# Minys233/GCN-BMP

Hardware: AMD Instinct MI355X
Metric: drug-pairs/sec fwd+bwd, binary-DDI GGNN d=128 (higher is better)
Workload: dtype f32; 1 GPU; C2: full binary DDI set (544 drugs, 147696 pairs), GGNN 4-step d=128 tied + Nie co-attention (head 8, tanh) + MLP(32,16), fwd+bwd+Adam, 1024 pairs/GPU/step, every molecule instance encoded; the 144 batches of one epoch resident in HBM, cycled; layout=per-instance packed layout, whole 128-row tiles, pairs_per_gpu=1024, global_batch=1024, parallelism=dp1

## Files before the change

gcn-bmp_amd/bmp/_lib.py:

```python
from __future__ import annotations

import ctypes
import os
from ctypes import c_float, c_int, c_size_t, c_void_p

import torch

_HERE = os.path.dirname(os.path.abspath(__file__))
LIB_PATH = os.environ.get("BMP_LIB_PATH") or os.path.join(_HERE, "libbmp_hip.so")

_P, _I, _Z, _F = c_void_p, c_int, c_size_t, c_float

SIGNATURES = {
    "bmp_version": (_I, []),
    "bmp_tile_rows": (_I, []),
    "bmp_prof_start": (_I, [_I]),
    "bmp_prof_stop": (_I, [_P]),
    "bmp_prof_collect": (_I, [_P, _P, _P, _P, _P, _I]),
    "bmp_stream_create_low": (_I, [_P]),
    "bmp_stream_destroy": (_I, [_P]),
    "bmp_embed_fwd": (_I, [_P, _P, _I, _I, _I, _P, _P]),
    "bmp_embed_bwd_ws_floats": (_Z, [_I, _I, _I]),
    "bmp_embed_bwd": (_I, [_P, _P, _I, _I, _I, _P, _P, _Z, _P]),
    "bmp_msg_fwd": (_I, [_P, _I, _I, _I, _I, _P, _P, _P, _P, _P, _P, _P, _I, _P, _P, _P, _I, _P]),
    "bmp_msg_bwd_ws_floats": (_Z, [_I, _I, _I]),
    "bmp_msg_bwd": (_I, [_P, _I, _P, _I, _I, _P, _I, _I, _I, _I, _P, _P, _P, _P, _P, _P, _P, _P, _P, _P, _P, _P, _I, _P, _P, _P, _Z, _P, _P]),
    "bmp_gru_fwd": (_I, [_P, _P, _I, _I, _I, _P, _P, _P, _P, _P, _P, _P]),
    "bmp_gru_bwd_ws_floats": (_Z, [_I, _I]),
    "bmp_gru_bwd": (_I, [_P, _P, _P, _P, _P, _I, _I, _I, _P, _P, _P, _P, _P, _P, _P, _I, _P, _Z, _P, _P]),
    "bmp_gru_state_fwd": (_I, [_P, _P, _P, _I, _I] + [_P] * 8),
    "bmp_gru_state_bwd_ws_floats": (_Z, [_I, _I]),
    "bmp_gru_state_bwd": (_I, [_P, _P, _P, _P, _P, _P, _I, _I] + [_P] * 11 + [_Z, _P]),
    "bmp_ggnn_step_supported": (_I, [_I]),
    "bmp_ggnn_step_fwd": (_I, [_P, _I, _I, _I, _I] + [_P] * 14 + [_I, _I, _P]),
    "bmp_ggnn_step_bwd": (_I, [_P, _P, _P, _P, _I, _I, _I] + [_P] * 10 + [_I, _I, _I, _P]),
    "bmp_step_wgrad_lists_used": (_I, [_I, _I]),
    "bmp_ggnn_step_wgrad_ws_floats": (_Z, [_I, _I]),
    "bmp_ggnn_step_wgrad": (_I, [_P, _P, _P, _P, _I, _I, _I, _P, _P, _P, _P, _I, _P, _P, _P, _P, _P, _Z, _P]),
    "bmp_type_rows_ws_ints": (_Z, [_I]),
    "bmp_type_rows": (_I, [_P, _P, _I, _P, _P, _P, _P]),
    "bmp_type_rows_live": (_I, [_P, _P, _P, _I, _P, _P, _P, _P]),
    "bmp_readout_tile_supported": (_I, [_I, _I, _I]),
    "bmp_readout_tile_fwd": (_I, [_P, _P, _I, _I, _P, _P, _I, _P, _P, _P, _P, _P, _P]),
    "bmp_relgcn_layer_supported": (_I, [_I, _I]),
    "bmp_relgcn_layer_fwd": (_I, [_P, _I, _I, _I, _P, _P, _P, _P, _P, _P, _P, _I, _P, _P, _P, _P, _I, _P]),
    "bmp_relgcn_layer_bwd": (_I, [_P, _P, _I, _I, _I, _P, _P, _P, _P, _P, _P, _P, _P, _P, _I, _I, _P]),
    "bmp_relgcn_layer_wgrad_ws_floats": (_Z, [_I, _I]),
    "bmp_relgcn_layer_wgrad": (_I, [_P, _P, _P, _I, _I, _P, _P, _P, _I, _P, _P, _P, _Z, _P]),
    "bmp_readout_fwd": (_I, [_P, _P, _I, _I, _I, _I, _P, _P, _I, _P, _P, _P, _I, _P, _P, _P]),
    "bmp_readout_bwd_ws_floats": (_Z, [_I, _I, _I, _I]),
    "bmp_readout_bwd": (_I, [_P, _P, _P, _I, _I, _I, _I, _P, _P, _I, _P, _P, _P, _I, _P, _P, _P, _P, _I, _P, _Z, _P, _P]),
    "bmp_linear_fwd": (_I, [_P, _I, _I, _I, _I, _P, _I, _P, _I, _P, _I, _P]),
    "bmp_wgrad_ws_floats_c": (_Z, [_I, _I, _I]),
    "bmp_linear_wgrad": (_I, [_P, _I, _P, _I, _I, _I, _I, _P, _P, _P, _Z, _P]),
    "bmp_segpool_fwd": (_I, [_P, _I, _P, _I, _P, _P, _P, _I, _P, _P]),
    "bmp_segpool_bwd": (_I, [_P, _P, _I, _P, _I, _P, _P, _P, _I, _I, _P, _P, _P]),
    "bmp_segsoftmax_fwd": (_I, [_P, _P, _P, _P, _I, _I, _P, _P]),
    "bmp_segsoftmax_bwd": (_I, [_P, _P, _P, _P, _P, _I, _I, _P, _P]),
    "bmp_rowbcast_fwd": (_I, [_P, _I, _P, _I, _P, _P]),
    "bmp_rowbcast_bwd": (_I, [_P, _I, _P, _P, _I, _P, _P]),
    "bmp_rowdot_fwd": (_I, [_P, _I, _P, _P, _P, _I, _P, _P]),
    "bmp_rowdot_bwd": (_I, [_P, _P, _I, _P, _P, _P, _P, _I, _I, _P, _P, _P, _P]),
    "bmp_rowcorr_fwd": (_I, [_P, _I, _P, _P, _P, _I, _P, _P]),
    "bmp_rowcorr_bwd": (_I, [_P, _P, _I, _P, _P, _P, _I, _P, _P, _P]),
    "bmp_dense_count": (_I, [_P, _I, _I, _P, _P, _P]),
    "bmp_dense_to_csr": (_I, [_P, _I, _I, _P, _P, _I, _P, _P, _P]),
    "bmp_collate_plan": (_I, [_P, _P, _I, _P, _P, _I, _P, _I, _P, _P, _P]),
    "bmp_collate_pair_meta": (_I, [_P, _I, _I, _I, _I, _P, _P, _P]),
# ... 104 lines not shown
```

gcn-bmp_amd/bmp/functional.py:

```python
from __future__ import annotations

import os

import torch
from torch.autograd import Function

from . import _lib
from ._lib import check, ptr, stream, require_rows
from .packed import PackedMolBatch

ACT = {"identity": 0, None: 0, "sigmoid": 1, "tanh": 2, "relu": 3}


def _ws(nfloats: int, device) -> torch.Tensor:
    return torch.empty(max(int(nfloats), 4), dtype=torch.float32, device=device)


def _check_pb(pb: PackedMolBatch, x: torch.Tensor) -> None:
    L = _lib.lib()
    if pb.R != L.bmp_tile_rows():
        raise ValueError(f"packed batch tile size R={pb.R} != library tile rows {L.bmp_tile_rows()}")
    if x.shape[0] != pb.n_rows:
        raise ValueError(f"row tensor has {x.shape[0]} rows, packed batch has {pb.n_rows}")

# ... 169 lines not shown
    tr = pb.type_rows_T(forward=forward)
    return tr if tr is not None else (None, None)


def step_lists(pb, N: int, d: int):
    tri, trc = type_rows(pb)
    if tri is None or not _lib.lib().bmp_step_wgrad_lists_used(int(N), int(d)):
        return None, None, 0
    return tri, trc, 1


def _rel_mt(pb):
    return (None, None) if pb.tile_stride else (pb.mt_row0, pb.mt_nblk)


def step_supported(d: int) -> bool:
    return bool(_lib.lib().bmp_ggnn_step_supported(int(d)))


def pack_k4(W: torch.Tensor) -> torch.Tensor:
    K, N = W.shape
    return W.detach().reshape(K // 4, 4, N).permute(0, 2, 1).contiguous()


def _cached(cache, tag, src, make):
    if cache is None:
        return make()
    key = (tag, src.data_ptr())
    if key not in cache:
        cache[key] = (make(), src)
    return cache[key][0]


class GGNNStepFn(Function):

    @staticmethod
    def forward(ctx, h, WT, bE, AT, UcT, b, pb, first, cache=None):
        L = _lib.lib()
        require_rows(h, "step: h")
        _check_pb(pb, h)
        N, d = h.shape
        if tuple(WT.shape) != (4 * d, d) or tuple(bE.shape) != (4, d) or tuple(AT.shape) != (2 * d, 3 * d) \
                or tuple(UcT.shape) != (d, d) or tuple(b.shape) != (3 * d,):
            raise ValueError("step: weight shapes do not match h")
        bE, b = bE.contiguous(), b.contiguous()
        WTp = _cached(cache, "f", WT, lambda: pack_k4(WT))
        ATp = _cached(cache, "f", AT, lambda: pack_k4(AT))
        UcTp = _cached(cache, "f", UcT, lambda: pack_k4(UcT))
        f = lambda *s: torch.empty(*s, dtype=torch.float32, device=h.device)
        m, rz, c, hout = f(N, d), f(N, 2 * d), f(N, d), f(N, d)
        check(L.bmp_ggnn_step_fwd(ptr(h), 0, pb.n_mtiles, d, int(first), ptr(pb.csr_ptr), ptr(pb.csr_col), ptr(pb.csr_val),
                                  ptr(WTp), ptr(bE), ptr(ATp), ptr(UcTp), ptr(b), ptr(m), ptr(rz), ptr(c), ptr(hout),
                                  ptr(pb.mt_row0), ptr(pb.mt_nblk), pb.n_rows, pb.tile_stride, stream()), "bmp_ggnn_step_fwd")
        ctx.save_for_backward(h, WT, AT, UcT, m, rz, c)
        ctx.pb, ctx.first, ctx.cache = pb, int(first), cache
        if cache is not None:
            key = ("n", WT.data_ptr(), AT.data_ptr())
            cache[key] = cache.get(key, 0) + 1
        return hout

    @staticmethod
    def backward(ctx, dhout):
        L = _lib.lib()
        h, WT, AT, UcT, m, rz, c = ctx.saved_tensors
        pb, first, cache = ctx.pb, ctx.first, ctx.cache
        N, d = h.shape
        dev = h.device
        dhout = dhout.contiguous()
        Wnat = _cached(cache, "b", WT, lambda: pack_k4(WT.t()))
        A = _cached(cache, "b", AT, lambda: pack_k4(AT.t()))
        Uc = _cached(cache, "b", UcT, lambda: pack_k4(UcT.t()))
        f = lambda *s: torch.empty(*s, dtype=torch.float32, device=dev)
        dh, gda = f(N, d), f(N, 7 * d)
        tri, trc, skip = step_lists(pb, N, d)
        check(L.bmp_ggnn_step_bwd(ptr(dhout), ptr(h), ptr(rz), ptr(c), pb.n_mtiles, d, first, ptr(pb.csrT_ptr),
                                  ptr(pb.csrT_col), ptr(pb.csrT_val), ptr(Wnat), ptr(A), ptr(Uc), ptr(dh), ptr(gda),
                                  ptr(pb.mt_row0), ptr(pb.mt_nblk), pb.n_rows, pb.tile_stride, skip, stream()), "bmp_ggnn_step_bwd")
        grp = ("g", WT.data_ptr(), AT.data_ptr())
        st = None
        if cache is not None and cache.get(("n",) + grp[1:], 1) > 1:
            st = cache.setdefault(grp, dict(seen=0, buf=None))
        if st is None or st["buf"] is None:
            o1, o2, dUcT, cs = f(d, 7 * d), f(d, 3 * d), f(d, d), f(7 * d)
            if st is not None:
                st["buf"] = (o1, o2, dUcT, cs)
        else:
            o1, o2, dUcT, cs = st["buf"]
        acc = 1 if (st is not None and st["seen"] > 0) else 0
        nws = L.bmp_ggnn_step_wgrad_ws_floats(N, d)
        ws = _ws(nws, dev)
        check(L.bmp_ggnn_step_wgrad(ptr(h), ptr(m), ptr(rz), ptr(gda), N, d, first, ptr(o1), ptr(o2), ptr(dUcT), ptr(cs),
                                    acc, ptr(tri), ptr(trc), None, None, ptr(ws), nws, stream()), "bmp_ggnn_step_wgrad")
        if st is not None:
            st["seen"] += 1
            if st["seen"] < cache[("n",) + grp[1:]]:
                return dh, None, None, None, None, None, None, None, None
            st["seen"], st["buf"] = 0, None
        dWT = o1[:, :4 * d].reshape(d, 4, d).permute(1, 0, 2).reshape(4 * d, d)
        dbE = cs[:4 * d].reshape(4, d)
        dAT = torch.cat((o1[:, 4 * d:], o2), dim=0)
        return dh, dWT, dbE, dAT, dUcT, cs[4 * d:], None, None, None


def flush_deferred_bwd(state) -> None:
    if state is not None and state.get("deferred_bwd"):
        fns = state["deferred_bwd"]
        state["deferred_bwd"] = []
        for fn in fns:
            fn()


def flush_deferred(state) -> None:
    if state is not None and state.get("deferred"):
        todo, state["deferred"] = state["deferred"], []
        for launch in todo:
            launch()


def _readout_fwd(h, h0, pb, WT, WTp, b, act_j, o, st=None, out=None, infer=False):
    L = _lib.lib()
    st = stream() if st is None else st
    N, d = h.shape
    d0 = 0 if h0 is None else h0.shape[1]
    tile = pb.row_mol is not None and not pb.oversized and bool(L.bmp_readout_tile_supported(d, d0, o))
    if out is not None:
        ij, g = out
    else:
        ij = None if (infer and tile) else torch.empty(N, 2 * o, dtype=torch.float32, device=h.device)
        g = torch.empty(pb.n_mols, o, dtype=torch.float32, device=h.device)
    if tile:
        if WTp is None:
            WTp = pack_k4(WT)
        check(L.bmp_readout_tile_fwd(ptr(h), ptr(h0), pb.n_tiles, d, ptr(WTp), ptr(b), act_j, ptr(pb.row_w), ptr(pb.row_mol),
                                     ptr(pb.mol_nrows), ptr(ij), ptr(g), st), "bmp_readout_tile_fwd")
# ... 175 lines not shown
        V, d = W.shape
        N = ids.numel()
        out = torch.empty(N, d, dtype=torch.float32, device=W.device)
        check(L.bmp_embed_fwd(ptr(ids), ptr(W), N, d, V, ptr(out), stream()), "bmp_embed_fwd")
        ctx.ids, ctx.dW, ctx.V, ctx.state = ids, dW, V, state
        _register(state, "embed.dW")
        return out

    @staticmethod
    def backward(ctx, dout):
        L = _lib.lib()
        dout = dout.contiguous()
        N, d = dout.shape
        nws = L.bmp_embed_bwd_ws_floats(N, d, ctx.V)
        ws = _ws(nws, dout.device)
        first = _first_write(ctx.state, "embed.dW")
        dst = ctx.dW if first else torch.empty_like(ctx.dW)
        check(L.bmp_embed_bwd(ptr(ctx.ids), ptr(dout), N, d, ctx.V, ptr(dst), ptr(ws), nws, stream()), "bmp_embed_bwd")
        if not first:
            ctx.dW.add_(dst)
        return None, None, None, None, None


def step_buffers(N: int, d: int, device, infer: bool = False):
    f = lambda *s: torch.empty(*s, dtype=torch.float32, device=device)
    if infer:
        return None, None, None, f(N, d)
    return f(N, d), f(N, 2 * d), f(N, d), f(N, d)


class PStepFn(Function):

    @staticmethod
    def forward(ctx, h, pb, W, G, state, gkey, first, bufs=None):
        L = _lib.lib()
        require_rows(h, "step: h")
        _check_pb(pb, h)
        N, d = h.shape
        m, rz, c, hout = bufs if bufs is not None else step_buffers(N, d, h.device)
        for t0, nt, st in _fwd_parts(state, pb, (h, m, rz, c, hout)):
            check(L.bmp_ggnn_step_fwd(ptr(h), t0, nt, d, int(first), ptr(pb.csr_ptr), ptr(pb.csr_col), ptr(pb.csr_val),
                                      ptr(W["WTp"]), ptr(W["bE"]), ptr(W["ATp"]), ptr(W["UcTp"]), ptr(W["b"]), ptr(m), ptr(rz),
                                      ptr(c), ptr(hout), ptr(pb.mt_row0), ptr(pb.mt_nblk), pb.n_rows, pb.tile_stride, st), "bmp_ggnn_step_fwd")
        ctx.save_for_backward(h, m, rz, c)
        ctx.pb, ctx.W, ctx.G, ctx.state, ctx.gkey, ctx.first = pb, W, G, state, gkey, int(first)
        if m is not None:
            type_rows(pb)
        _register(state, gkey)
        return hout

    @staticmethod
    def backward(ctx, dhout):
        L = _lib.lib()
        h, m, rz, c = ctx.saved_tensors
        pb, W, G, first = ctx.pb, ctx.W, ctx.G, ctx.first
        N, d = h.shape
        dhout = dhout.contiguous()
        dh = torch.empty(N, d, dtype=torch.float32, device=h.device)
        gda = torch.empty(N, 7 * d, dtype=torch.float32, device=h.device)
        tri, trc, skip = step_lists(pb, N, d)
        lvi, lvc = pb._cache.get("live_rows", (None, None)) if tri is not None else (None, None)
        check(L.bmp_ggnn_step_bwd(ptr(dhout), ptr(h), ptr(rz), ptr(c), pb.n_mtiles, d, first, ptr(pb.csrT_ptr),
                                  ptr(pb.csrT_col), ptr(pb.csrT_val), ptr(W["Wnat_p"]), ptr(W["A_p"]), ptr(W["Uc_p"]),
                                  ptr(dh), ptr(gda), ptr(pb.mt_row0), ptr(pb.mt_nblk), pb.n_rows, pb.tile_stride, skip, stream()), "bmp_ggnn_step_bwd")
        acc = 0 if _first_write(ctx.state, ctx.gkey) else 1

        def wgrad(st, ws_of):
            nws = L.bmp_ggnn_step_wgrad_ws_floats(N, d)
            ws = ws_of(nws, h.device)
            check(L.bmp_ggnn_step_wgrad(ptr(h), ptr(m), ptr(rz), ptr(gda), N, d, first, ptr(G["o1"]), ptr(G["o2"]),
                                        ptr(G["dUcT"]), ptr(G["cs"]), acc, ptr(tri), ptr(trc), ptr(lvi), ptr(lvc), ptr(ws), nws, st), "bmp_ggnn_step_wgrad")

        _on_side(ctx.state, (h, m, rz, gda), wgrad)
        return dh, None, None, None, None, None, None, None


def _ptr_array(tensors):
    import ctypes
    return (ctypes.c_void_p * len(tensors))(*[None if t is None else t.data_ptr() for t in tensors])


class PReadoutFn(Function):

    @staticmethod
    def forward(ctx, h, h0, pb, W, G, act_j, state, off_chain=False, infer=False):
        L = _lib.lib()
        require_rows(h, "readout: h")
        _check_pb(pb, h)
        N, d = h.shape
        d0 = 0 if h0 is None else h0.shape[1]
        ctx.state = state
        WT = W["WT"]
        o = WT.shape[1] // 2
        side = state.get("side") if (off_chain and state is not None and _RO_OFF_CHAIN) else None
        ctx.off_chain = side is not None
        if side is not None:
            tile = pb.row_mol is not None and not pb.oversized and bool(L.bmp_readout_tile_supported(d, d0, o))
            ij = None if tile else torch.empty(N, 2 * o, dtype=torch.float32, device=h.device)
            g = torch.empty(pb.n_mols, o, dtype=torch.float32, device=h.device)

            sp = state.get("split")

            def launch():
                if sp is not None:
                    sp.stream.wait_stream(torch.cuda.current_stream())
                    _readout_fwd(h, h0, pb, WT, W.get("WTp"), W.get("b"), act_j, o, sp.handle, out=(ij, g))
                    state.setdefault("split_keep", []).append((h, h0, ij, g))
# ... 213 lines not shown
```

gcn-bmp_amd/bmp/ggnn.py:

```python
from __future__ import annotations

import math
from typing import Optional

import numpy as np
import torch
from torch import nn

from . import functional as Fn
from .packed import PackedMolBatch, pack_from_dense

MAX_ATOMIC_NUM = 117
NUM_EDGE_TYPE = 4


class Linear(nn.Module):

    def __init__(self, in_size: Optional[int], out_size: int, nobias: bool = False):
        super().__init__()
        if in_size is None:
            self.W = nn.UninitializedParameter()
        else:
            self.W = nn.Parameter(torch.randn(out_size, in_size) / math.sqrt(in_size))
        self.b = None if nobias else nn.Parameter(torch.zeros(out_size))
# ... 296 lines not shown
        self.atoms = PackedAtoms(h, pb, 0 if pb.dense_map is not None else None)
        return self._readout_fast(h, h0, pb, fast)

    def _readout_fast(self, h, h0, pb, fast):
        P, G, state, _tape = fast
        infer = not torch.is_grad_enabled()
        if not self._plan_fused():
            return Fn.PReadoutFn.apply(h, h0, pb, dict(WT=P["ro.WT"], b=P["ro.b"], Wnat=P["ro.Wnat"]),
                                       dict(dWT=G["ro.dWT"], db=G["ro.db"]), Fn.ACT["identity"], state,
                                       getattr(self, "_readout_off_chain", False))
        return Fn.PReadoutFn.apply(h, h0, pb, dict(WT=P["ro.WT"], b=P["ro.b"], Wnat=P["ro.Wnat"], WTp=P.get("ro.WTp")),
                                   dict(dWT=G["ro.dWT"], db=G["ro.db"]), Fn.ACT["identity"], state,
                                   getattr(self, "_readout_off_chain", False), infer)

    def _encode_fast(self, pb, fast, h_in=None):
        P, G, state, tape = fast
        if h_in is None:
            pb.check_atom_ids(P["embed.W"].shape[0])
            h = Fn.PEmbedFn.apply(tape, P["embed.W"], pb.atom_id, G["embed.dW"], state)
        else:
            h = h_in
        h0 = h
        if not self._plan_fused():
            for step, (li, mode) in enumerate(self._step_groups()):
                Wm = dict(WT=P[f"msg{li}.WT"], bE=P[f"msg{li}.bE"], Wnat=P[f"msg{li}.Wnat"])
                m = Fn.PMsgFn.apply(h, pb, Wm, dict(dWT=G[f"msg{li}.dWT"], dbE=G[f"msg{li}.dbE"]), state, f"msg{li}", Fn.ACT["identity"])
                Wg = dict(AT=P[f"gru_{mode}.AT"], UcT=P["gru.UcT"], b=P[f"gru_{mode}.b"], A=P[f"gru_{mode}.A"], Uc=P["gru.Uc"])
                Gg = dict(dAT=G[f"gru_{mode}.dAT"], dUcT=G[f"gru_{mode}.dUcT"], db=G[f"gru_{mode}.db"])
                h = Fn.PGRUFn.apply(h, m, pb, Wg, Gg, state, f"gru_{mode}", step == 0)
            Fn._join_parts(state)
            return h, h0
        infer = not torch.is_grad_enabled()
        bufs = [Fn.step_buffers(h.shape[0], self.hidden_dim, h.device, infer) for _ in range(self.n_layers)]
        Fn.fork_parts(state, pb)
        per_step = getattr(self, "_per_step", None)
        if per_step is None or per_step[0] is not P:
            lst = []
            for step, (li, mode) in enumerate(self._step_groups()):
                W = dict(WTp=P[f"msg{li}.WTp"], bE=P[f"msg{li}.bE"], Wnat_p=P[f"msg{li}.Wnat_p"], ATp=P[f"gru_{mode}.ATp"],
                         b=P[f"gru_{mode}.b"], A_p=P[f"gru_{mode}.A_p"], UcTp=P["gru.UcTp"], Uc_p=P["gru.Uc_p"])
                g = f"g{li}_{mode}"
                Gs = dict(o1=G[g + ".o1"], o2=G[g + ".o2"], dUcT=G[g + ".dUcT"], cs=G[g + ".cs"])
                lst.append((W, Gs, g, step == 0))
            per_step = (P, lst)
            object.__setattr__(self, "_per_step", per_step)
        per_step = per_step[1]
        for step, (W, Gs, g, first) in enumerate(per_step):
            h = Fn.PStepFn.apply(h, pb, W, Gs, state, g, first, bufs[step])
        Fn._join_parts(state)
        return h, h0

    def encode_rows(self, pb: PackedMolBatch):
        if self.concat_hidden or (self.dropout_rate != 0.0 and self.training):
            raise NotImplementedError("encode_rows: concat_hidden / training dropout take the per-instance batch form")
        fast = getattr(self, "_fast", None)
        if fast is not None and not pb.oversized:
            return self._encode_fast(pb, fast)
        pb.check_atom_ids(self.embed.W.shape[0])
        h = Fn.EmbedFn.apply(self.embed.W, pb.atom_id)
        h0 = h
        fused = self.fused and self._plan_fused() and not pb.oversized
        later, msgw, cache = None, {}, {}
        for step in range(self.n_layers):
            li = 0 if self.weight_tying else step
            if li not in msgw:
                msgw[li] = message_kernel_weights(self.message_layers[li])
            WT, bE = msgw[li]
            if step == 0:
                AT, UcT, b = self.update_layer.kernel_weights(first=True)
            else:
                if later is None:
                    later = self.update_layer.kernel_weights(first=False)
                AT, UcT, b = later
            if fused:
                h = Fn.GGNNStepFn.apply(h, WT, bE, AT, UcT, b, pb, step == 0, cache)
            else:
                m = Fn.MsgFn.apply(h, WT, bE, None, None, pb, Fn.ACT["identity"])
                h = Fn.GRUFn.apply(h, m, AT, UcT, b, pb, step == 0)
        return h, h0

    def readout_rows(self, h, h0, pb: PackedMolBatch):
        fast = getattr(self, "_fast", None)
        if fast is not None and not pb.oversized:
            return self._readout_fast(h, h0, pb, fast)
        return self.readout(h, h0, pb, 0)

    def forward(self, atom_array, adj=None):
        drop = self.dropout_rate != 0.0 and self.training
        dev = self.embed.W.device
        h_in = None
        if _is_float_atoms(atom_array):
            pb, h_in = pack_float_atoms(atom_array, adj, dev)
            if h_in.shape[1] != self.hidden_dim:
                raise ValueError(f"float atom features must be hidden_dim={self.hidden_dim} wide, got {h_in.shape[1]}")
        else:
            pb = as_packed(atom_array, adj, dev)
        fast = getattr(self, "_fast", None)
        big = pb.oversized
        if fast is not None and not drop and not big:
            return self._forward_fast(pb, fast, h_in)
        if h_in is None:
            pb.check_atom_ids(self.embed.W.shape[0])
        h = Fn.EmbedFn.apply(self.embed.W, pb.atom_id) if h_in is None else h_in
        h0 = h
        later = None
        fused = self.fused and self._plan_fused() and not drop and not big
        state, state_w = None, None
        masks = getattr(self, "_dropout_masks", None)
        g_list = []
        msgw, cache = {}, {}
        for step in range(self.n_layers):
            li = 0 if self.weight_tying else step
            if li not in msgw:
                msgw[li] = message_kernel_weights(self.message_layers[li])
            WT, bE = msgw[li]
            if step == 0:
                AT, UcT, b = self.update_layer.kernel_weights(first=True)
            else:
                if later is None:
                    later = self.update_layer.kernel_weights(first=False)
                AT, UcT, b = later
            if fused:
                h = Fn.GGNNStepFn.apply(h, WT, bE, AT, UcT, b, pb, step == 0, cache)
            elif drop:
                m = Fn.MsgFn.apply(h, WT, bE, None, None, pb, Fn.ACT["identity"])
                if state is None:
                    state = Fn.GRUFn.apply(h, m, AT, UcT, b, pb, True)
                else:
                    if state_w is None:
                        state_w = self.update_layer.kernel_weights_state()
                    state = Fn.GRUStateFn.apply(h, m, state, *state_w, pb)
                if masks is not None:
                    h = state * masks[step]
                else:
                    h = torch.nn.functional.dropout(state, p=self.dropout_rate, training=True)
            else:
                m = Fn.MsgFn.apply(h, WT, bE, None, None, pb, Fn.ACT["identity"])
                h = Fn.GRUFn.apply(h, m, AT, UcT, b, pb, step == 0)
            if self.concat_hidden:
                g_list.append(self.readout(h, h0, pb, step))
        self.atoms = PackedAtoms(h, pb, 0 if pb.dense_map is not None else None)
        if self.concat_hidden:
            return torch.cat(g_list, dim=1)
        return self.readout(h, h0, pb, 0)

    def get_atom_array(self):
        assert self.atoms is not None
        return self.atoms
```

gcn-bmp_amd/csrc/bmp_ops.hip:

```cpp
#include <string.h>
#include "bmp_kernels.h"

static inline RGArgs rg_zero() {
    RGArgs a;
    memset(&a, 0, sizeof(a));
    return a;
}

static inline size_t max_sz(size_t a, size_t b) { return a > b ? a : b; }

__global__ void k_dact(const float* __restrict__ dout, int lddo, const float* __restrict__ out, int ldo, int act, int N,
                       int d, float* __restrict__ dpre) {
    const size_t total = (size_t)N * d;
    for (size_t idx = (size_t)blockIdx.x * blockDim.x + threadIdx.x; idx < total; idx += (size_t)gridDim.x * blockDim.x) {
        const int row = (int)(idx / d), c = (int)(idx % d);
        dpre[idx] = dout[(size_t)row * lddo + c] * bmp_dact(act, out[(size_t)row * ldo + c]);
    }
}

__global__ void k_gru_bwd_gates(const float* __restrict__ dhn, const float* __restrict__ h, const float* __restrict__ rz,
                                const float* __restrict__ c, int N, int d, int first, float* __restrict__ da,
                                float* __restrict__ dhacc) {
    const size_t total = (size_t)N * d;
    for (size_t idx = (size_t)blockIdx.x * blockDim.x + threadIdx.x; idx < total; idx += (size_t)gridDim.x * blockDim.x) {
// ... 423 lines not shown
        WGArgs g{h, nullptr, d, 0, dij, 2 * o, d, 2 * o, N, dWT, 2 * o, acc, db};
        if ((rc = bmp_launch_wgrad(g, slab, st_w))) return rc;
        if (h0) {
            WGArgs g2{h0, nullptr, d0, 0, dij, 2 * o, d0, 2 * o, N, dWT + (size_t)d * 2 * o, 2 * o, acc};
            if ((rc = bmp_launch_wgrad(g2, slab, st_w))) return rc;
        }
    }
    return 0;
}

extern "C" int bmp_linear_fwd(const float* X, int ldx, int n_tiles, int K, int Nout, const float* WT, int ldw,
                              const float* b, int act, float* Y, int ldy, hipStream_t st) {
    RGArgs a = rg_zero();
    a.s[0] = RGSrc{X, nullptr, WT, ldx, 0, ldw, K};
    a.nsrc = 1; a.Nout = Nout; a.Y = Y; a.ldy = ldy; a.bias = b;
    a.act_lo = a.act_hi = act;
    return bmp_launch_rowgemm(a, n_tiles, BMP_EPI_GENERIC, st);
}

extern "C" size_t bmp_wgrad_ws_floats_c(int N, int K, int Nn) {
    return max_sz(bmp_wgrad_ws_floats(N, K, Nn), bmp_colsum_ws_floats(N, Nn));
}

extern "C" int bmp_linear_wgrad(const float* X, int ldx, const float* dY, int ldy, int N, int K, int Nn, float* dWT,
                                float* db, float* ws, size_t ws_floats, hipStream_t st) {
    BMP_REQUIRE(ws_floats >= bmp_wgrad_ws_floats_c(N, K, Nn));
    WGArgs g{X, nullptr, ldx, 0, dY, ldy, K, Nn, N, dWT, Nn, 0};
    int rc = bmp_launch_wgrad(g, ws, st);
    if (rc) return rc;
    if (db) return bmp_launch_colsum(dY, ldy, N, Nn, db, 0, ws, st);
    return 0;
}

extern "C" int bmp_version(void) { return 408; }
extern "C" int bmp_tile_rows(void) { return BMP_R; }
```

include/bmp.h:

```cpp
#ifndef BMP_H_
#define BMP_H_
#include <stddef.h>

#ifdef __cplusplus
extern "C" {
#endif

typedef struct ihipStream_t* bmp_stream_t;

enum { BMP_ACT_NONE = 0, BMP_ACT_SIGMOID = 1, BMP_ACT_TANH = 2, BMP_ACT_RELU = 3 };

int bmp_version(void);
int bmp_tile_rows(void);

int bmp_prof_start(int kclass);
int bmp_prof_stop(double* out);
int bmp_prof_collect(int* key, int* count, double* ms, double* flops, double* bytes, int cap);

int bmp_stream_create_low(bmp_stream_t* out);
int bmp_stream_destroy(bmp_stream_t stream);

int bmp_embed_fwd(const int* ids, const float* W, int N, int d, int V, float* out, bmp_stream_t stream);
size_t bmp_embed_bwd_ws_floats(int N, int d, int V);
int bmp_embed_bwd(const int* ids, const float* dout, int N, int d, int V, float* dW, float* ws, size_t ws_floats,
// ... 2 lines not shown
int bmp_msg_fwd(const float* x, int ldx, int n_tiles, int d_in, int d_out, const int* csr_ptr, const int* csr_col,
                const float* csr_val, const float* WT, const float* bE, const float* WsT, const float* bs, int act,
                float* agg, float* wdeg, float* out, int ldo, bmp_stream_t stream);
size_t bmp_msg_bwd_ws_floats(int n_tiles, int d_in, int d_out);
int bmp_msg_bwd(const float* dout, int lddo, const float* out, int ldo, int act, const float* x, int ldx, int n_tiles,
                int d_in, int d_out, const int* csrT_ptr, const int* csrT_col, const float* csrT_val, const float* Wnat,
                const float* Ws, const float* agg, const float* wdeg, float* dx, float* dWT, float* dbE, float* dWsT,
                float* dbs, int accumulate_w, const int* type_rows_f, const int* type_cnt_f, float* ws, size_t ws_floats,
                bmp_stream_t stream, bmp_stream_t stream_w);

int bmp_gru_fwd(const float* h, const float* m, int n_tiles, int d, int first, const float* AT, const float* UcT,
                const float* b, float* rz, float* c, float* hout, bmp_stream_t stream);
size_t bmp_gru_bwd_ws_floats(int n_tiles, int d);
int bmp_gru_bwd(const float* dhout, const float* h, const float* m, const float* rz, const float* c, int n_tiles, int d,
                int first, const float* A, const float* Uc, float* dh, float* dm, float* dAT, float* dUcT, float* db,
                int accumulate_w, float* ws, size_t ws_floats, bmp_stream_t stream, bmp_stream_t stream_w);

int bmp_gru_state_fwd(const float* hd, const float* m, const float* s, int n_tiles, int d, const float* WT, const float* UrzT,
                      const float* UcT, const float* b, float* rz, float* c, float* sout, bmp_stream_t stream);
size_t bmp_gru_state_bwd_ws_floats(int n_tiles, int d);
int bmp_gru_state_bwd(const float* dsout, const float* hd, const float* m, const float* s, const float* rz, const float* c,
                      int n_tiles, int d, const float* A, const float* Urz, const float* Uc, float* dhd, float* dm, float* ds,
                      float* dWT, float* dUrzT, float* dUcT, float* db, float* ws, size_t ws_floats, bmp_stream_t stream);

int bmp_ggnn_step_supported(int d);
int bmp_ggnn_step_fwd(const float* h, int tile0, int n_tiles, int d, int first, const int* csr_ptr, const int* csr_col,
                      const float* csr_val, const float* WT, const float* bE, const float* AT, const float* UcT,
                      const float* b, float* m, float* rz, float* c, float* hout, const int* mt_row0, const int* mt_nblk,
                      int mt_rows, int tile_stride, bmp_stream_t stream);
int bmp_ggnn_step_bwd(const float* dhout, const float* h, const float* rz, const float* c, int n_tiles, int d, int first,
                      const int* csrT_ptr, const int* csrT_col, const float* csrT_val, const float* Wnat, const float* A,
                      const float* Uc, float* dh, float* gda, const int* mt_row0, const int* mt_nblk, int mt_rows, int tile_stride,
                      int skip_zero_g, bmp_stream_t stream);
int bmp_step_wgrad_lists_used(int N, int d);
size_t bmp_ggnn_step_wgrad_ws_floats(int N, int d);
int bmp_ggnn_step_wgrad(const float* h, const float* m, const float* rz, const float* gda, int N, int d, int first,
                        float* o1, float* o2, float* dUcT, float* cs, int accumulate, const int* type_rows, const int* type_cnt,
                        const int* live_rows, const int* live_cnt, float* ws, size_t ws_floats, bmp_stream_t stream);

size_t bmp_type_rows_ws_ints(int N);
int bmp_type_rows(const int* csr_ptr, const int* csr_col, int N, int* idx, int* cnt, int* ws, bmp_stream_t stream);
int bmp_type_rows_live(const int* csr_ptr, const int* csr_col, const int* row_mol, int N, int* idx, int* cnt, int* ws,
                       bmp_stream_t stream);

int bmp_relgcn_layer_supported(int d_in, int d_out);
int bmp_relgcn_layer_fwd(const float* h, int tile0, int n_tiles, int d, const int* csr_ptr, const int* csr_col, const float* csr_val,
                         const float* WT, const float* bE, const float* WsT, const float* bs, int act, float* out,
                         float* wdeg, const int* mt_row0, const int* mt_nblk, int mt_rows, bmp_stream_t stream);
int bmp_relgcn_layer_bwd(const float* dout, const float* out, int act, int n_tiles, int d, const int* csrT_ptr,
                         const int* csrT_col, const float* csrT_val, const float* Wnat, const float* Ws, float* dh,
                         float* gda, const int* mt_row0, const int* mt_nblk, int mt_rows, int skip_zero_g, bmp_stream_t stream);
size_t bmp_relgcn_layer_wgrad_ws_floats(int N, int d);
int bmp_relgcn_layer_wgrad(const float* h, const float* wdeg, const float* gda, int N, int d, float* o1, float* dbE,
                           float* cs, int accumulate, const int* type_rows, const int* type_cnt, float* ws, size_t ws_floats,
                           bmp_stream_t stream);

int bmp_readout_fwd(const float* h, const float* h0, int n_tiles, int d, int d0, int o, const float* WT, const float* b,
                    int act_j, const float* row_w, const int* mol_row0, const int* mol_nrows, int n_mols, float* ij,
                    float* g, bmp_stream_t stream);
size_t bmp_readout_bwd_ws_floats(int n_tiles, int d, int d0, int o);
int bmp_readout_bwd(const float* dg, const float* h, const float* h0, int n_tiles, int d, int d0, int o,
                    const float* Wnat, const float* ij, int act_j, const float* row_w, const int* mol_row0,
                    const int* mol_nrows, int n_mols, float* dh, float* dh0, float* dWT, float* db, int accumulate_w,
                    float* ws, size_t ws_floats, bmp_stream_t stream, bmp_stream_t stream_w);
int bmp_readout_tile_supported(int d, int d0, int o);
int bmp_readout_tile_fwd(const float* h, const float* h0, int n_tiles, int d, const float* WT, const float* b, int act_j,
// ... 123 lines not shown
```

Before: 405,800 pairs/s.

## Precompute per-atom-type tables for first GGNN step from embedding

When the first step's input is an embedding lookup, the atom-type embeddings are multiplied once by the message weights and the first-step GRU input weights, giving a V×6d table. The first-step kernel then gathers table rows by atom id instead of running dense GEMMs for the message transform and the z/c input projections, leaving only the second half of the GRU matmul. This adds a small per-call table kernel and an indirect gather path, and duplicates logic in a new kernel that must stay consistent with the existing step.

```diff
diff --git a/gcn-bmp_amd/bmp/_lib.py b/gcn-bmp_amd/bmp/_lib.py
--- a/gcn-bmp_amd/bmp/_lib.py
+++ b/gcn-bmp_amd/bmp/_lib.py
@@ -34,6 +34,9 @@
     "bmp_ggnn_step_supported": (_I, [_I]),
     "bmp_ggnn_step_fwd": (_I, [_P, _I, _I, _I, _I] + [_P] * 14 + [_I, _I, _P]),
     "bmp_ggnn_step_bwd": (_I, [_P, _P, _P, _P, _I, _I, _I] + [_P] * 10 + [_I, _I, _I, _P]),
+    "bmp_ggnn_first_tables_floats": (_Z, [_I, _I]),
+    "bmp_ggnn_first_tables": (_I, [_P, _I, _I, _P, _P, _P, _P]),
+    "bmp_ggnn_step_first_fwd": (_I, [_P, _P, _I, _I, _I, _I] + [_P] * 12 + [_I, _I, _P]),
     "bmp_step_wgrad_lists_used": (_I, [_I, _I]),
     "bmp_ggnn_step_wgrad_ws_floats": (_Z, [_I, _I]),
     "bmp_ggnn_step_wgrad": (_I, [_P, _P, _P, _P, _I, _I, _I, _P, _P, _P, _P, _I, _P, _P, _P, _P, _P, _Z, _P]),
diff --git a/gcn-bmp_amd/bmp/functional.py b/gcn-bmp_amd/bmp/functional.py
--- a/gcn-bmp_amd/bmp/functional.py
+++ b/gcn-bmp_amd/bmp/functional.py
@@ -225,10 +225,23 @@
     return cache[key][0]
 
 
+def first_tables_supported(d: int) -> bool:
+    return int(d) in (64, 128)
+
+
+def first_tables(embW: torch.Tensor, WTp: torch.Tensor, ATp: torch.Tensor, st=None) -> torch.Tensor:
+    L = _lib.lib()
+    V, d = embW.shape
+    tab = torch.empty(L.bmp_ggnn_first_tables_floats(V, d), dtype=torch.float32, device=embW.device)
+    check(L.bmp_ggnn_first_tables(ptr(embW), V, d, ptr(WTp), ptr(ATp), ptr(tab), stream() if st is None else st),
+          "bmp_ggnn_first_tables")
+    return tab
+
+
 class GGNNStepFn(Function):
 
     @staticmethod
-    def forward(ctx, h, WT, bE, AT, UcT, b, pb, first, cache=None):
+    def forward(ctx, h, WT, bE, AT, UcT, b, pb, first, cache=None, emb=None):
         L = _lib.lib()
         require_rows(h, "step: h")
         _check_pb(pb, h)
@@ -242,9 +255,17 @@
         UcTp = _cached(cache, "f", UcT, lambda: pack_k4(UcT))
         f = lambda *s: torch.empty(*s, dtype=torch.float32, device=h.device)
         m, rz, c, hout = f(N, d), f(N, 2 * d), f(N, d), f(N, d)
-        check(L.bmp_ggnn_step_fwd(ptr(h), 0, pb.n_mtiles, d, int(first), ptr(pb.csr_ptr), ptr(pb.csr_col), ptr(pb.csr_val),
-                                  ptr(WTp), ptr(bE), ptr(ATp), ptr(UcTp), ptr(b), ptr(m), ptr(rz), ptr(c), ptr(hout),
-                                  ptr(pb.mt_row0), ptr(pb.mt_nblk), pb.n_rows, pb.tile_stride, stream()), "bmp_ggnn_step_fwd")
+        if emb is not None and first and first_tables_supported(d):
+            embW, ids = emb
+            embW = embW.detach().contiguous()
+            tab = first_tables(embW, WTp, ATp)
+            check(L.bmp_ggnn_step_first_fwd(ptr(ids), ptr(tab), embW.shape[0], 0, pb.n_mtiles, d, ptr(pb.csr_ptr), ptr(pb.csr_col),
+                                            ptr(pb.csr_val), ptr(bE), ptr(ATp), ptr(b), ptr(m), ptr(rz), ptr(c), ptr(hout),
+                                            ptr(pb.mt_row0), ptr(pb.mt_nblk), pb.n_rows, pb.tile_stride, stream()), "bmp_ggnn_step_first_fwd")
+        else:
+            check(L.bmp_ggnn_step_fwd(ptr(h), 0, pb.n_mtiles, d, int(first), ptr(pb.csr_ptr), ptr(pb.csr_col), ptr(pb.csr_val),
+                                      ptr(WTp), ptr(bE), ptr(ATp), ptr(UcTp), ptr(b), ptr(m), ptr(rz), ptr(c), ptr(hout),
+                                      ptr(pb.mt_row0), ptr(pb.mt_nblk), pb.n_rows, pb.tile_stride, stream()), "bmp_ggnn_step_fwd")
         ctx.save_for_backward(h, WT, AT, UcT, m, rz, c)
         ctx.pb, ctx.first, ctx.cache = pb, int(first), cache
         if cache is not None:
@@ -287,12 +308,12 @@
         if st is not None:
             st["seen"] += 1
             if st["seen"] < cache[("n",) + grp[1:]]:
-                return dh, None, None, None, None, None, None, None, None
+                return dh, None, None, None, None, None, None, None, None, None
             st["seen"], st["buf"] = 0, None
         dWT = o1[:, :4 * d].reshape(d, 4, d).permute(1, 0, 2).reshape(4 * d, d)
         dbE = cs[:4 * d].reshape(4, d)
         dAT = torch.cat((o1[:, 4 * d:], o2), dim=0)
-        return dh, dWT, dbE, dAT, dUcT, cs[4 * d:], None, None, None
+        return dh, dWT, dbE, dAT, dUcT, cs[4 * d:], None, None, None, None
 
 
 def flush_deferred_bwd(state) -> None:
@@ -534,13 +555,21 @@
 class PStepFn(Function):
 
     @staticmethod
-    def forward(ctx, h, pb, W, G, state, gkey, first, bufs=None):
+    def forward(ctx, h, pb, W, G, state, gkey, first, bufs=None, tabs=None):
         L = _lib.lib()
         require_rows(h, "step: h")
         _check_pb(pb, h)
         N, d = h.shape
         m, rz, c, hout = bufs if bufs is not None else step_buffers(N, d, h.device)
-        for t0, nt, st in _fwd_parts(state, pb, (h, m, rz, c, hout)):
+        if tabs is not None and not first:
+            raise ValueError("step: the table form is the first step's")
+        for t0, nt, st in _fwd_parts(state, pb, (h, m, rz, c, hout, tabs)):
+            if tabs is not None:
+                ids, tab, V = tabs
+                check(L.bmp_ggnn_step_first_fwd(ptr(ids), ptr(tab), V, t0, nt, d, ptr(pb.csr_ptr), ptr(pb.csr_col), ptr(pb.csr_val),
+                                                ptr(W["bE"]), ptr(W["ATp"]), ptr(W["b"]), ptr(m), ptr(rz), ptr(c), ptr(hout),
+                                                ptr(pb.mt_row0), ptr(pb.mt_nblk), pb.n_rows, pb.tile_stride, st), "bmp_ggnn_step_first_fwd")
+                continue
             check(L.bmp_ggnn_step_fwd(ptr(h), t0, nt, d, int(first), ptr(pb.csr_ptr), ptr(pb.csr_col), ptr(pb.csr_val),
                                       ptr(W["WTp"]), ptr(W["bE"]), ptr(W["ATp"]), ptr(W["UcTp"]), ptr(W["b"]), ptr(m), ptr(rz),
                                       ptr(c), ptr(hout), ptr(pb.mt_row0), ptr(pb.mt_nblk), pb.n_rows, pb.tile_stride, st), "bmp_ggnn_step_fwd")
@@ -574,7 +603,7 @@
                                         ptr(G["dUcT"]), ptr(G["cs"]), acc, ptr(tri), ptr(trc), ptr(lvi), ptr(lvc), ptr(ws), nws, st), "bmp_ggnn_step_wgrad")
 
         _on_side(ctx.state, (h, m, rz, gda), wgrad)
-        return dh, None, None, None, None, None, None, None
+        return dh, None, None, None, None, None, None, None, None
 
 
 def _ptr_array(tensors):
diff --git a/gcn-bmp_amd/bmp/ggnn.py b/gcn-bmp_amd/bmp/ggnn.py
--- a/gcn-bmp_amd/bmp/ggnn.py
+++ b/gcn-bmp_amd/bmp/ggnn.py
@@ -352,6 +352,10 @@
             return h, h0
         infer = not torch.is_grad_enabled()
         bufs = [Fn.step_buffers(h.shape[0], self.hidden_dim, h.device, infer) for _ in range(self.n_layers)]
+        tabs = None
+        if h_in is None and Fn.first_tables_supported(self.hidden_dim):
+            embW = P["embed.W"]
+            tabs = (pb.atom_id, Fn.first_tables(embW, P["msg0.WTp"], P["gru_first.ATp"]), embW.shape[0])
         Fn.fork_parts(state, pb)
         per_step = getattr(self, "_per_step", None)
         if per_step is None or per_step[0] is not P:
@@ -366,7 +370,7 @@
             object.__setattr__(self, "_per_step", per_step)
         per_step = per_step[1]
         for step, (W, Gs, g, first) in enumerate(per_step):
-            h = Fn.PStepFn.apply(h, pb, W, Gs, state, g, first, bufs[step])
+            h = Fn.PStepFn.apply(h, pb, W, Gs, state, g, first, bufs[step], tabs if step == 0 else None)
         Fn._join_parts(state)
         return h, h0
 
@@ -393,7 +397,7 @@
                     later = self.update_layer.kernel_weights(first=False)
                 AT, UcT, b = later
             if fused:
-                h = Fn.GGNNStepFn.apply(h, WT, bE, AT, UcT, b, pb, step == 0, cache)
+                h = Fn.GGNNStepFn.apply(h, WT, bE, AT, UcT, b, pb, step == 0, cache, (self.embed.W, pb.atom_id) if step == 0 else None)
             else:
                 m = Fn.MsgFn.apply(h, WT, bE, None, None, pb, Fn.ACT["identity"])
                 h = Fn.GRUFn.apply(h, m, AT, UcT, b, pb, step == 0)
@@ -441,7 +445,8 @@
                     later = self.update_layer.kernel_weights(first=False)
                 AT, UcT, b = later
             if fused:
-                h = Fn.GGNNStepFn.apply(h, WT, bE, AT, UcT, b, pb, step == 0, cache)
+                h = Fn.GGNNStepFn.apply(h, WT, bE, AT, UcT, b, pb, step == 0, cache,
+                                        (self.embed.W, pb.atom_id) if (step == 0 and h_in is None) else None)
             elif drop:
                 m = Fn.MsgFn.apply(h, WT, bE, None, None, pb, Fn.ACT["identity"])
                 if state is None:
diff --git a/gcn-bmp_amd/csrc/bmp_first.hip b/gcn-bmp_amd/csrc/bmp_first.hip
--- /dev/null
+++ b/gcn-bmp_amd/csrc/bmp_first.hip
@@ -0,0 +1,199 @@
+#include <string.h>
+#include "bmp_kernels.h"
+#include "bmp_tile.h"
+
+__global__ __launch_bounds__(256) void k_first_tables(const float* __restrict__ embW, int V, int d, const float* __restrict__ WT,
+                                                      const float* __restrict__ AT, float* __restrict__ tab) {
+    __shared__ __attribute__((aligned(16))) float w[128];
+    const int v = blockIdx.x;
+    for (int k = threadIdx.x; k < d; k += 256) w[k] = embW[(size_t)v * d + k];
+    __syncthreads();
+    for (int n = threadIdx.x; n < 6 * d; n += 256) {
+        const float* B; int ldn, kb, nc;
+        if (n < 4 * d) { B = WT; ldn = d; kb = (n / d) * d; nc = n % d; }
+        else { B = AT; ldn = 3 * d; kb = 0; nc = n - 3 * d; }
+        float s = 0.f;
+        for (int k = 0; k < d; k += 4) {
+            const f32x4 b4 = *(const f32x4*)(B + ((size_t)((kb + k) >> 2) * ldn + nc) * 4);
+            const f32x4 w4 = *(const f32x4*)(w + k);
+#pragma unroll
+            for (int t = 0; t < 4; ++t) s = __builtin_fmaf(w4[t], b4[t], s);
+        }
+        if (n < 4 * d) tab[(size_t)v * 4 * d + n] = s;
+        else tab[(size_t)V * 4 * d + (size_t)v * 2 * d + (n - 4 * d)] = s;
+    }
+}
+
+struct FirstArgs {
+    const int* ptr; const int* col; const float* val;
+    int tile0;
+    const int* mt_row0; const int* mt_nblk;
+    int tile_stride;
+    const int* atom_id;
+    const float* TW;
+    const float* TA;
+    int V;
+    const float* bE;
+    const float* AT;
+    const float* b;
+    float* m; float* rz; float* c; float* hout;
+};
+
+template <int D>
+__device__ __forceinline__ void first_msg_row(f32x4 (&acc)[D / 16], const int* ptr, const int* col, const float* val, const int* ids,
+                                              const float* TW, const float* bE, int V, int row0, int row, int q) {
+    constexpr int F = D / 16;
+#pragma unroll
+    for (int f = 0; f < F; ++f) acc[f] = (f32x4){0.f, 0.f, 0.f, 0.f};
+    float wd[4] = {0.f, 0.f, 0.f, 0.f};
+    const int e0 = ptr[row], e1 = ptr[row + 1];
+    for (int ed = e0; ed < e1; ++ed) {
+        const int cv = col[ed];
+        const float v = val[ed];
+        const int e = cv & 3;
+        int j = ids[((cv >> 2) - row0) & (FZ_R - 1)];
+        j = j < 0 ? 0 : (j >= V ? V - 1 : j);
+        const float* s = TW + (size_t)j * 4 * D + e * D + q * (D / 4);
+#pragma unroll
+        for (int f = 0; f < F; ++f) acc[f] += *(const f32x4*)(s + 4 * f) * v;
+#pragma unroll
+        for (int t = 0; t < 4; ++t) wd[t] += (e == t) ? v : 0.f;
+    }
+#pragma unroll
+    for (int f = 0; f < F; ++f) {
+        f32x4 be[4];
+#pragma unroll
+        for (int t = 0; t < 4; ++t) be[t] = *(const f32x4*)(bE + t * D + q * (D / 4) + 4 * f);
+#pragma unroll
+        for (int x = 0; x < 4; ++x)
+            acc[f][x] = __builtin_fmaf(wd[3], be[3][x], __builtin_fmaf(wd[2], be[2][x], __builtin_fmaf(wd[1], be[1][x],
+                                       __builtin_fmaf(wd[0], be[0][x], acc[f][x]))));
+    }
+}
+
+template <int D, bool VAR, bool SAVE>
+__global__ __launch_bounds__(512) void k_ggnn_first_fwd(FirstArgs a) {
+    constexpr int LD = D + 4;
+    constexpr int NCB = D / 32, NRW = 8 / NCB, RB = 4 / NRW;
+    extern __shared__ __attribute__((aligned(16))) float lds[];
+    float* As = lds;
+    int* ids = (int*)(As + FZ_R * LD);
+    int* rptr = ids + FZ_R;
+    int* ecol = rptr + 132;
+    float* evalv = (float*)(ecol + FZ_ECAP);
+    int* sy = (int*)(evalv + FZ_ECAP);
+
+    const int tid = threadIdx.x, lane = tid & 63, w = tid >> 6;
+    const int grp = w >> 2;
+    GrpSync gs{sy + grp, 0};
+    if (tid < 2) sy[tid] = 0;
+    const int wc = w % NCB, wr = w / NCB;
+    const int l31 = lane & 31, hi = lane >> 5;
+    FZ_TILE_SETUP();
+    if (VAR && a.tile_stride > nrows) {
+        const int e = row0 + a.tile_stride;
+        fz_clear_rows<512>(a.hout, D, row0 + nrows, e, tid);
+        fz_clear_rows<512>(a.m, D, row0 + nrows, e, tid);
+        fz_clear_rows<512>(a.rz, 2 * D, row0 + nrows, e, tid);
+        fz_clear_rows<512>(a.c, D, row0 + nrows, e, tid);
+    }
+    const int col = wc * 32 + l31;
+    const int wrow0 = wr * RB * 32;
+    const int lrow = wrow0 + 4 * hi;
+    const int rot = (tile * 8) % D;
+    const float* Aw = As + (wrow0 + l31) * LD + 4 * hi;
+
+    if (tid < nrows) ids[tid] = a.atom_id[row0 + tid];
+    const bool csr_lds = stage_csr(a.ptr, a.col, a.val, row0, rptr, ecol, evalv, nrows);
+    const int ldwg[2] = {3 * D, 3 * D};
+    const float* const base_m = a.AT + (size_t)(D + 4 * hi) * 3 * D + 4 * col + 4 * D;
+    const float* const Bm[2] = {base_m, base_m + 4 * D};
+    BPre<2> pre_m;
+    tile_b_prefetch<2>(pre_m, Bm, ldwg, D, rot);
+    __syncthreads();
+    if (!grp_live) return;
+
+    {
+        const int row = tid >> 2, q = tid & 3;
+        if (row < nrows) {
+            f32x4 acc[D / 16];
+            if (csr_lds) first_msg_row<D>(acc, rptr, ecol, evalv, ids, a.TW, a.bE, a.V, row0, row, q);
+            else first_msg_row<D>(acc, a.ptr + row0, a.col, a.val, ids, a.TW, a.bE, a.V, row0, row, q);
+            float* o = As + row * LD + q * (D / 4);
+#pragma unroll
+            for (int f = 0; f < D / 16; ++f) *(f32x4*)(o + 4 * f) = acc[f];
+            if (SAVE) {
+                float* g = a.m + (size_t)(row0 + row) * D + q * (D / 4);
+#pragma unroll
+                for (int f = 0; f < D / 16; ++f) *(f32x4*)(g + 4 * f) = acc[f];
+            }
+        }
+    }
+    f32x16 gg[2][RB];
+    zero_acc(gg[0]); zero_acc(gg[1]);
+    FZ_FOR_ACC {
+        int j = ids[lrow + rb * 32 + (reg & 3) + 8 * (reg >> 2)];
+        j = j < 0 ? 0 : (j >= a.V ? a.V - 1 : j);
+        const float* t = a.TA + (size_t)j * 2 * D + col;
+        gg[0][rb][reg] = t[0];
+        gg[1][rb][reg] = t[D];
+    }
+    FZ_GSYNC();
+    tile_mma_n<VAR, 2, RB>(nrb, gg, Aw, LD, Bm, ldwg, D, rot, &pre_m);
+    {
+        const float bz = a.b[D + col], bcn = a.b[2 * D + col];
+        const AccBuf rzo = acc_buf<2 * D>(a.rz, row0, lrow, col);
+        const AccBuf co = acc_buf<D>(a.c, row0, lrow, col);
+        const AccBuf ho = acc_buf<D>(a.hout, row0, lrow, col);
+        FZ_FOR_ACC {
+            const float zv = bmp_sigmoid(gg[0][rb][reg] + bz);
+            const float cv = bmp_tanh(gg[1][rb][reg] + bcn);
+            if (SAVE) { acc_st<2 * D>(rzo, rb, reg, zv, D); acc_st<D>(co, rb, reg, cv); }
+            acc_st<D>(ho, rb, reg, zv * cv);
+        }
+    }
+}
+
+static size_t first_lds_bytes(int D) { return ((size_t)FZ_R * (D + 4) + FZ_R + 132 + 2 * FZ_ECAP + 2) * sizeof(float); }
+
+template <int D, bool VAR>
+static int first_launch(const FirstArgs& a, int n_tiles, double rows, hipStream_t st) {
+    const bool keep = a.m != nullptr;
+    const void* fn = keep ? (const void*)k_ggnn_first_fwd<D, VAR, true> : (const void*)k_ggnn_first_fwd<D, VAR, false>;
+    if (int rc_attr = bmp_lds_attr(fn, first_lds_bytes(D))) return rc_attr;
+    BmpProfScope prof(BMP_KCLS_STEP_FWD, 2.0 * rows * 8.0 * D * D, 4.0 * rows * (D * 4.0 + 1.0), st, BMP_KID_GGNN_FIRST);
+    if (keep) hipLaunchKernelGGL((k_ggnn_first_fwd<D, VAR, true>), dim3(n_tiles), dim3(512), first_lds_bytes(D), st, a);
+    else hipLaunchKernelGGL((k_ggnn_first_fwd<D, VAR, false>), dim3(n_tiles), dim3(512), first_lds_bytes(D), st, a);
+    BMP_LAUNCH_CHECK();
+    return 0;
+}
+
+extern "C" size_t bmp_ggnn_first_tables_floats(int V, int d) { return (size_t)V * 6 * d; }
+
+extern "C" int bmp_ggnn_first_tables(const float* embW, int V, int d, const float* WT, const float* AT, float* tab, hipStream_t st) {
+    BMP_REQUIRE(embW && WT && AT && tab && V > 0 && (d == 64 || d == 128));
+    BMP_REQUIRE(((uintptr_t)WT & 15) == 0 && ((uintptr_t)AT & 15) == 0);
+    hipLaunchKernelGGL(k_first_tables, dim3(V), dim3(256), 0, st, embW, V, d, WT, AT, tab);
+    BMP_LAUNCH_CHECK();
+    return 0;
+}
+
+extern "C" int bmp_ggnn_step_first_fwd(const int* atom_id, const float* tab, int V, int tile0, int n_tiles, int d,
+                                       const int* csr_ptr, const int* csr_col, const float* csr_val, const float* bE,
+                                       const float* AT, const float* b, float* m, float* rz, float* c, float* hout,
+                                       const int* mt_row0, const int* mt_nblk, int mt_rows, int tile_stride, hipStream_t st) {
+    BMP_REQUIRE(tile0 >= 0 && n_tiles > 0 && V > 0 && (d == 64 || d == 128));
+    BMP_REQUIRE(atom_id && tab && csr_ptr && csr_col && csr_val && bE && AT && b && hout);
+    BMP_REQUIRE(((uintptr_t)tab & 15) == 0 && ((uintptr_t)AT & 15) == 0 && ((uintptr_t)bE & 15) == 0);
+    BMP_REQUIRE((mt_row0 != nullptr) == (mt_nblk != nullptr));
+    BMP_REQUIRE(tile_stride == 0 || (tile_stride == FZ_R && mt_row0 != nullptr));
+    BMP_REQUIRE((m != nullptr) == (rz != nullptr) && (m != nullptr) == (c != nullptr));
+    BMP_REQUIRE(m == nullptr || (((uintptr_t)m & 15) == 0));
+    FirstArgs a; memset(&a, 0, sizeof(a));
+    a.ptr = csr_ptr; a.col = csr_col; a.val = csr_val; a.tile0 = tile0; a.mt_row0 = mt_row0; a.mt_nblk = mt_nblk;
+    a.tile_stride = tile_stride; a.atom_id = atom_id; a.TW = tab; a.TA = tab + (size_t)V * 4 * d; a.V = V;
+    a.bE = bE; a.AT = AT; a.b = b; a.m = m; a.rz = rz; a.c = c; a.hout = hout;
+    const double rows = mt_row0 != nullptr ? (double)mt_rows : (double)n_tiles * FZ_R;
+    if (mt_row0 != nullptr) return d == 128 ? first_launch<128, true>(a, n_tiles, rows, st) : first_launch<64, true>(a, n_tiles, rows, st);
+    return d == 128 ? first_launch<128, false>(a, n_tiles, rows, st) : first_launch<64, false>(a, n_tiles, rows, st);
+}
diff --git a/gcn-bmp_amd/csrc/bmp_ops.hip b/gcn-bmp_amd/csrc/bmp_ops.hip
--- a/gcn-bmp_amd/csrc/bmp_ops.hip
+++ b/gcn-bmp_amd/csrc/bmp_ops.hip
@@ -479,5 +479,5 @@
     return 0;
 }
 
-extern "C" int bmp_version(void) { return 408; }
+extern "C" int bmp_version(void) { return 409; }
 extern "C" int bmp_tile_rows(void) { return BMP_R; }
diff --git a/include/bmp.h b/include/bmp.h
--- a/include/bmp.h
+++ b/include/bmp.h
@@ -58,6 +58,12 @@
                       const int* csrT_ptr, const int* csrT_col, const float* csrT_val, const float* Wnat, const float* A,
                       const float* Uc, float* dh, float* gda, const int* mt_row0, const int* mt_nblk, int mt_rows, int tile_stride,
                       int skip_zero_g, bmp_stream_t stream);
+size_t bmp_ggnn_first_tables_floats(int V, int d);
+int bmp_ggnn_first_tables(const float* embW, int V, int d, const float* WT, const float* AT, float* tab, bmp_stream_t stream);
+int bmp_ggnn_step_first_fwd(const int* atom_id, const float* tab, int V, int tile0, int n_tiles, int d, const int* csr_ptr,
+                            const int* csr_col, const float* csr_val, const float* bE, const float* AT, const float* b,
+                            float* m, float* rz, float* c, float* hout, const int* mt_row0, const int* mt_nblk, int mt_rows,
+                            int tile_stride, bmp_stream_t stream);
 int bmp_step_wgrad_lists_used(int N, int d);
 size_t bmp_ggnn_step_wgrad_ws_floats(int N, int d);
 int bmp_ggnn_step_wgrad(const float* h, const float* m, const float* rz, const float* gda, int N, int d, int first,
```

Measured after the change: 411,800 pairs/s (median of 6 runs). 1.01x the previous value.
